# HalfSummer11/CAPTRA

Measured on AMD Instinct MI355X. Metric: tracked frames/sec (4096-pt clouds), higher is better.
Workload: dtype f32; 1 GPU; NOCS-REAL275-shaped rigid category 'bottle' (1 part, symmetric), 4096 pts/frame, batch=32 trajectories per GPU, fp32 (BASELINE.json configs[1]); points=4096, trajectories_per_gpu=32, distinct_clouds_per_gpu=32, parallelism=dp1 (trajectory-sharded, RCCL all-gather of poses), weights=seeded default_rng(7), real architecture (3.96 M params), physical-regime plants

## Files before the change

captra_amd/_lib.py:

```python
from __future__ import annotations

import contextlib
import ctypes as C
import threading
import os
from pathlib import Path

import torch

_PKG = Path(__file__).resolve().parent
LIB_PATH = Path(os.environ["CAPTRA_LIB"]) if os.environ.get("CAPTRA_LIB") else _PKG / "lib" / "libcaptra_hip.so"

_lib = None

_INT, _LL, _F, _P = C.c_int, C.c_longlong, C.c_float, C.c_void_p

_SIGNATURES = {
    "captra_furthest_point_sampling": [_INT, _INT, _INT, _P, _P, _P, _P],
    "captra_ball_query": [_INT, _INT, _INT, _F, _INT, _P, _P, _P, _P],
    "captra_group_points": [_INT, _INT, _INT, _INT, _INT, _P, _P, _P, _P],
    "captra_group_points_multi": [_INT, _INT, _INT, _P, _P, _P, _P, _P, _P, _P],
    "captra_group_points_grad": [_INT, _INT, _INT, _INT, _INT, _P, _P, _P, _P],
    "captra_group_points_grad_ws": [_INT, _INT, _INT, _INT, _INT, _P, _P, _P, _P, C.c_size_t, _P],
    "captra_three_interpolate_grad_ws": [_INT, _INT, _INT, _INT, _P, _P, _P, _P, _P, C.c_size_t, _P],
# ... 100 lines not shown
    "captra_packed_weight_floats": ([_INT, _INT], _LL),
    "captra_dense_bf16_image_bytes": ([_INT, _INT], _LL),
    "captra_gn_stats_bf16pm_tiles": ([_LL], _INT),
    "captra_dense_bf16_stats_tiles": ([_LL], _INT),
    "captra_dense_bf16_tile_stats_tiles": ([_LL], _INT),
    "captra_chain_bf16_image_bytes": ([_INT, _INT], _LL),
    "captra_dense_x6_image_bytes": ([_INT, _INT], _LL),
    "captra_sa_x6_image_bytes": ([_INT] * 4, _LL),
    "captra_chain_x6_image_bytes": ([_INT, _P, _P], _LL),
    "captra_sa_bf16_image_bytes": ([_INT] * 4, _LL),
    "captra_sa1_stream_scratch_bytes": ([_INT, _INT], _LL),
    "captra_sa1_stream_set_grid": ([_INT, _INT], None),
    "captra_sa1_stream_set_fine": ([_INT], None),
    "captra_sa1_stream_set_whole": ([_INT], None),
    "captra_neck_chain_set_split": ([_INT], None),
    "captra_image_members_set_split": ([_INT], None),
    "captra_query_and_group_set_shape": ([_INT, _INT], None),
    "captra_pointwise_mlp_gn_tiles": ([_INT, _INT, _LL], _INT),
    "captra_pointwise_mlp_gn_tiles_ex": ([_INT, _INT, _LL, _P], _INT),
}

_ENV_SWITCHES = {
    "CAPTRA_BF16_SHARED_AFFINE": ("captra_dense_bf16_set_shared_affine", ()),
    "CAPTRA_SA_BF16_VARIANT": ("captra_sa_bf16_set_variant", ()),
    "CAPTRA_FPS_DEFER": ("captra_fps_set_defer", ()),
    "CAPTRA_NN_SPLIT": ("captra_three_nn_set_split", ()),
    "CAPTRA_BQ_CPW": ("captra_ball_query_set_cpw", ()),
    "CAPTRA_SA_SPLIT": ("captra_sa_fused_set_split", ()),
    "CAPTRA_HEAD_PERSIST": ("captra_tile_bf16_set_persistent", ()),
    "CAPTRA_L1_FINE": ("captra_sa1_stream_set_fine", ()),
    "CAPTRA_L1_WHOLE": ("captra_sa1_stream_set_whole", ()),
    "CAPTRA_L1_GRID": ("captra_sa1_stream_set_grid", (1,)),
}


class CaptraHipError(RuntimeError):
    pass


class LaunchOpts(C.Structure):
    _fields_ = [("splitk_positions", _INT), ("sa_prezeroed", _INT), ("centre_m0", _INT), ("centre_mc", _INT), ("reserved_cus", _INT),
                ("dyn_slot", _P)]

# ... 146 lines not shown
```

captra_amd/csrc/sa_fused.hip:

```cpp
#include "common.h"
#include "wave_mlp.h"

namespace {


constexpr int SF_POS = 128;
constexpr int SF_BK = 16;
constexpr int SF_BM = 128;
constexpr int SF_MAXC = 256;

struct SaParams {
    int n, m, k, cfeat;
    int c1, c2, c3;
    const float *feat;
    const float *xyz_cn;
    const float *new_xyz;
    const int *idx;
    const float *w1, *b1, *w2, *b2, *w3, *b3;
    float *out;
    int out_ctotal, co_off;
};

template <int WN>
__device__ __forceinline__ void sa_prefetch_first(float (&pre)[16], const float *__restrict__ wt, int cin, int cout) {
// ... 222 lines not shown
    }
}

struct SwParams {
    int b, n, m, k;
    const float *feat, *xyz_cn, *new_xyz;
    const int *idx;
    const float *w1, *b1, *w2, *b2, *w3, *b3;
    float *out;
    int out_ctotal, co_off;
    const float *v1;
    unsigned long long *prof;
    int split;
    int m0, mc;
    int *dyn;
};

#define SW_TICK(slot)                                                         \
    if (CAPTRA_PROF_ON(p.prof)) {                                                  \
        const unsigned long long t_now = __builtin_amdgcn_s_memtime();        \
        if (lane == 0 && sampled) atomicAdd(p.prof + (slot), t_now - t_last); \
        t_last = t_now;                                                       \
    }

template <int CF, int C1, int NOUT, typename Next>
__device__ __forceinline__ void sw_layer1_gather(const SwParams &p, int b, int id, const float (&ctr)[3], const float *bias_lds,
                                                 float (&hout)[NOUT], int lane, Next next) {
    constexpr int CIN = CF + 3;
    using S = SwShape<CIN, C1>;
    constexpr int NT = S::NT;
// ... 240 lines not shown
#undef SL_LOAD_QUAD
#pragma unroll
        for (int tm = 0; tm < 2; ++tm)
            if (2 * ps + tm < S::NT) {
                if (LAST) sw_bfly_accumulate(acc[tm], zrun[2 * ps + tm], lane);
                else sw_mid_epilogue<NOUT>(acc[tm], 2 * ps + tm, hout);
            }
    }
}

template <int CF, int C1, int C2, int C3>
constexpr int sl_lds_floats() {
    return SlShape<CF + 3, C1>::FLOATS + SlShape<C1, C2>::FLOATS + SlShape<C2, C3>::FLOATS + pad32c(C1) + pad32c(C2) + pad32c(C3);
}

template <int CF, int C1, int C2, int C3>
__device__ __forceinline__ void sl_body(const SwParams &p, const int blk, const int nblk) {
    constexpr int CIN1 = CF + 3;
    static_assert(CIN1 <= 8, "LDS-weight variant is for the small-input scales");
    using S1 = SlShape<CIN1, C1>;
    using S2 = SlShape<C1, C2>;
    using S3 = SlShape<C2, C3>;
    extern __shared__ __attribute__((aligned(16))) float lds[];
    float *wl1 = lds, *wl2 = wl1 + S1::FLOATS, *wl3 = wl2 + S2::FLOATS;
    float *bias1 = wl3 + S3::FLOATS, *bias2 = bias1 + pad32c(C1), *bias3 = bias2 + pad32c(C2);
    const int tid = threadIdx.x, lane = tid & 63;
    const int wave = __builtin_amdgcn_readfirstlane(tid >> 6);

    const int nwaves = nblk * SL_WAVES, gid = blk * SL_WAVES + wave;
    const int ncentres = p.b * p.mc;
// ... 14 lines not shown
            else if (row < CIN1) v = p.xyz_cn[((size_t)tb * 3 + (row - CF)) * p.n + id_] - (row - CF == 0 ? c_[0] : (row - CF == 1 ? c_[1] : c_[2]));
            x_[j] = v;
        }
    };
    const bool split = p.split != 0;
    const int ssh = __builtin_ctz((unsigned)nslices);
    int task = gid;
    int c = split ? gid >> ssh : gid, sl = split ? gid & (nslices - 1) : 0;
    int c_next = gid + nwaves;
    const bool dyn = p.dyn != nullptr && !split && nslices > 1;
    int dyn_raw = 0;
    if (dyn) {
        if (lane == 0) dyn_raw = atomicAdd(p.dyn, 1);
        c = __builtin_amdgcn_readfirstlane(dyn_raw);
    }
    int id = 0;
    float ctr[3] = {0.f, 0.f, 0.f};
    if (c < ncentres) {
        id = load_ids(c, sl);
        load_ctr(c, ctr);
    }
    sl_stage_weights<CIN1, C1>(wl1, p.w1, tid);
    sl_stage_weights<C1, C2>(wl2, p.w2, tid);
    sl_stage_weights<C2, C3>(wl3, p.w3, tid);
    for (int e = tid; e < pad32c(C1); e += SL_WAVES * 64) bias1[e] = p.b1[e];
    for (int e = tid; e < pad32c(C2); e += SL_WAVES * 64) bias2[e] = p.b2[e];
    for (int e = tid; e < pad32c(C3); e += SL_WAVES * 64) bias3[e] = p.b3[e];
    __syncthreads();

    float x1[S1::KST];
#pragma unroll
    for (int j = 0; j < S1::KST; ++j) x1[j] = 0.f;
    if (c < ncentres) gather_x1(c, id, ctr, x1);
    int zrun[S3::NT];
    const bool sampled = blk % 16 == 0;
    unsigned long long t_last = CAPTRA_PROF_ON(p.prof) ? __builtin_amdgcn_s_memtime() : 0ull;
    while (c < ncentres) {
        if (sl == 0 || split) {
#pragma unroll
            for (int t = 0; t < S3::NT; ++t) zrun[t] = 0;
        }
        const bool last_slice = split || sl + 1 == nslices;
        if (dyn) {
            if (sl == 0 && lane == 0) dyn_raw = atomicAdd(p.dyn, 1);
            if (last_slice) c_next = __builtin_amdgcn_readfirstlane(dyn_raw);
        }
        const int cn = split ? (task + nwaves) >> ssh : (last_slice ? c_next : c), sn = split ? (task + nwaves) & (nslices - 1) : (last_slice ? 0 : sl + 1);
        const bool has_next = cn < ncentres;
        int id_n = 0;
        float ctr_n[3] = {ctr[0], ctr[1], ctr[2]};
        if (has_next) {
            id_n = load_ids(cn, sn);
            if (last_slice) load_ctr(cn, ctr_n);
        }
        float h1[S2::KST], h2[S3::KST], none[1];
        float x1_n[S1::KST];
#pragma unroll
        for (int j = 0; j < S1::KST; ++j) x1_n[j] = 0.f;
        SW_TICK(0)
        sl_layer<CIN1, C1, false>(wl1, bias1, x1, h1, zrun, lane);
        SW_TICK(1)
        sl_layer<C1, C2, false>(wl2, bias2, h1, h2, zrun, lane);
        if (has_next) gather_x1(cn, id_n, ctr_n, x1_n);
        SW_TICK(2)
        sl_layer<C2, C3, true>(wl3, bias3, h2, none, zrun, lane);
        SW_TICK(3)
        if (CAPTRA_PROF_ON(p.prof) && lane == 0 && sampled) atomicAdd(p.prof + 9, 1ull);
        if (last_slice) {
            const int tb = c / p.mc, centre = p.m0 + c - tb * p.mc;
            const int r = lane & 15;
            const int row0 = 8 * (r >> 2) + (r & 3) + 4 * (lane >> 5);
            float *op = p.out + ((size_t)tb * p.out_ctotal + p.co_off + row0) * p.m + centre;
#pragma unroll
            for (int t = 0; t < S3::NT; ++t) {
                const float v = sw_bfly_finish(zrun[t]);
                if ((lane & 16) == 0 && 32 * t + row0 < C3) {
                    if (split) atomicMax(reinterpret_cast<int *>(op + (size_t)32 * t * p.m), __float_as_int(v));
                    else op[(size_t)32 * t * p.m] = v;
                }
            }
            if (!dyn) c_next += nwaves;
// ... 18 lines not shown
    const int blk = (int)blockIdx.x;
    if (blk < q.g0) sl_body<CF, 32, 32, 64>(q.s[0], blk, q.g0);
    else if (blk < q.g0 + q.g1) sl_body<CF, 64, 64, 128>(q.s[1], blk - q.g0, q.g1);
    else sl_body<CF, 64, 96, 128>(q.s[2], blk - q.g0 - q.g1, (int)gridDim.x - q.g0 - q.g1);
}

}

static CAPTRA_KNOB int g_sa_wn = 0;
extern "C" void captra_sa_fused_set_wn(int wn) { g_sa_wn = wn; }
static CAPTRA_KNOB int g_sa_mode = 0;
extern "C" void captra_sa_fused_set_mode(int mode) { g_sa_mode = mode; }
static CAPTRA_KNOB int g_sa_split = 1;
extern "C" void captra_sa_fused_set_split(int v) { g_sa_split = v; }
int captra_sa_split_knob() { return g_sa_split; }
struct SlRecord {
    SwParams q;
    unsigned grid;
    int code, cf, lds;
    void (*launch)(const SwParams &, unsigned, int, hipStream_t);
};
struct SlCollect {
    SlRecord rec[3];
    int n = 0;
    alignas(16) unsigned char sp[1024];
};
template <int CF, int C1, int C2, int C3>
static void sl_launch_one(const SwParams &q, unsigned grid, int lds, hipStream_t s) {
    CAPTRA_LAUNCH("sa_scale_fused", (sa_wave_lds_kernel<CF, C1, C2, C3>), dim3(grid), dim3(SL_WAVES * 64), lds, s, q);
}
// ... 50 lines not shown
                               const float *w3, const float *b3, float *out, int out_ctotal, int co_off,
                               const captra_launch_opts *opts, SlCollect *col, captra_stream_t stream) {
    if (b < 0 || n < 1 || m < 0 || k < 1 || cfeat < 0 || c1 < 1 || c2 < 1 || c3 < 1) return -1;
    if (cfeat > 0 && feat == nullptr) return -1;
    if (out_ctotal < co_off + c3 || co_off < 0) return -1;
    if (k % 32 != 0 || 128 % k != 0 || c1 > SF_MAXC || c2 > SF_MAXC || c3 > SF_MAXC) return -2;
    if (b == 0 || m == 0) return 0;
    SaParams p;
    p.n = n; p.m = m; p.k = k; p.cfeat = cfeat; p.c1 = c1; p.c2 = c2; p.c3 = c3;
    p.feat = feat; p.xyz_cn = xyz_cn; p.new_xyz = new_xyz; p.idx = idx;
    p.w1 = w1; p.b1 = b1; p.w2 = w2; p.b2 = b2; p.w3 = w3; p.b3 = b3;
    p.out = out; p.out_ctotal = out_ctotal; p.co_off = co_off; 
    if (g_sa_mode != 1) {
        SwParams q;
        q.b = b; q.n = n; q.m = m; q.k = k; q.feat = feat; q.xyz_cn = xyz_cn; q.new_xyz = new_xyz; q.idx = idx;
        q.w1 = w1; q.b1 = b1; q.w2 = w2; q.b2 = b2; q.w3 = w3; q.b3 = b3; q.out = out; q.out_ctotal = out_ctotal; q.co_off = co_off; q.v1 = nullptr; q.prof = g_sa_prof; q.split = 0; q.dyn = nullptr;
        const long long Lw = (long long)m * k;
        dim3 gridw((unsigned)((Lw + SF_POS - 1) / SF_POS), b);
#define SL_CASE(CF_, C1_, C2_, C3_)                                                                                   \
    if (g_sa_mode != 2 && cfeat == CF_ && c1 == C1_ && c2 == C2_ && c3 == C3_ && k % 32 == 0 && (long long)b * m < (1ll << 30)) { \
        constexpr auto kern = sa_wave_lds_kernel<CF_, C1_, C2_, C3_>;                                                  \
        constexpr int lds_bytes = sl_lds_floats<CF_, C1_, C2_, C3_>() * 4;                                             \
        if (int e = captra_allow_lds<kern>(lds_bytes)) return e;                                                       \
         \
        const int resident = captra_blocks_per_cu<kern>(SL_WAVES * 64, lds_bytes) * captra_free_cus(opts);             \
        int wm0, wmc;                                                                                                  \
        (void)captra_centre_window(opts, m, &wm0, &wmc);                                                               \
        if (wmc == 0) return 0;                                                                                        \
        q.m0 = wm0; q.mc = wmc;                                                                                        \
        const long long centres = (long long)b * wmc;                     \
         \
// ... 92 lines not shown
    const int ferr = sl_collect_flush(col, (hipStream_t)stream);
    return err != 0 ? err : ferr;
}

extern "C" int captra_sa_scale_pre(int b, int n, int m, int k, int cfeat, int c1, int c2, int c3, const float *v1,
                                   const float *xyz_cn, const float *new_xyz, const int *idx, const float *w1,
                                   const float *w2, const float *b2, const float *w3, const float *b3, float *out,
                                   int out_ctotal, int co_off, captra_stream_t stream) {
    if (b < 0 || n < 1 || m < 0 || k < 1 || cfeat < 1 || c1 < 1 || c2 < 1 || c3 < 1 || v1 == nullptr) return -1;
    if (out_ctotal < co_off + c3 || co_off < 0) return -1;
    if (k % 32 != 0 || 128 % k != 0) return -2;
    if ((long long)c1 * n * 4 >= (1ll << 31)) return -2;
    SwParams q;
    q.b = b; q.n = n; q.m = m; q.k = k; q.feat = nullptr; q.xyz_cn = xyz_cn; q.new_xyz = new_xyz; q.idx = idx;
    q.w1 = w1; q.b1 = b2 ; q.w2 = w2; q.b2 = b2; q.w3 = w3; q.b3 = b3;
    q.out = out; q.out_ctotal = out_ctotal; q.co_off = co_off; q.v1 = v1; q.prof = g_sa_prof; q.split = 0; q.dyn = nullptr;
    const long long Lw = (long long)m * k;
    dim3 gridw((unsigned)((Lw + SF_POS - 1) / SF_POS), b);
#define SWP_CASE(CF_, C1_, C2_, C3_)                                                                                       \
    if (cfeat == CF_ && c1 == C1_ && c2 == C2_ && c3 == C3_) {                                                             \
        if (b == 0 || m == 0) return 0;                                                                                    \
        CAPTRA_LAUNCH("sa_scale_fused", (sa_wave_kernel<CF_, C1_, C2_, C3_, true>), gridw, dim3(256), 0, (hipStream_t)stream, q); \
        return captra_last_error();                                                                                        \
    }
    SWP_CASE(320, 128, 128, 256)
    SWP_CASE(320, 128, 196, 256)
#undef SWP_CASE
    return -2;
}
```

captra_amd/csrc/sa_pipe.hip:

```cpp
#include "wave_mlp.h"

namespace {

constexpr int SP_POS = 128;

struct SpParams {
    int b, n, m, k;
    const float *v1pm;
    const float *xyz_cn;
    const float *new_xyz;
    const int *idx;
    const float *w1;
    const float *w2, *b2, *w3, *b3;
    float *out;
    int out_ctotal, co_off;
    unsigned long long *prof;
    int split;
    int *dyn;
};

#define SP_TICK(slot)                                                           \
    if (CAPTRA_PROF_ON(p.prof)) {                                                    \
        const unsigned long long t_now = __builtin_amdgcn_s_memtime();          \
        if (lane == 0 && sampled) atomicAdd(p.prof + (slot), t_now - t_last);   \
        t_last = t_now;                                                         \
    }

template <int NOUT>
__device__ __forceinline__ void sp_mid_unit(const f32x16 &acc, int t, int q, float (&hout)[NOUT]) {
    unsigned a[4];
#pragma unroll
    for (int i = 0; i < 4; ++i) {
        const int x = __float_as_int(acc[4 * q + i]);
// ... 145 lines not shown
    float at[2][NT1];
    {
        const __amdgpu_buffer_rsrc_t rw = __builtin_amdgcn_make_buffer_rsrc((void *)p.w1, 0, S1::KP * S1::LDW * 4, 0x00020000);
        const int voff_w = (half * S1::LDW + (lane & 31)) * 4;
#pragma unroll
        for (int jj = 0; jj < 2; ++jj)
#pragma unroll
            for (int t = 0; t < NT1; ++t)
                at[jj][t] = __builtin_bit_cast(float, __builtin_amdgcn_raw_buffer_load_b32(rw, voff_w, ((CF + 2 * jj) * S1::LDW + 32 * t) * 4, 0));
    }
    __syncthreads();

    const int nwaves = nblk * 4, gid = blk * 4 + wave;
    const int ncentres = p.b * p.m;
    const int nslices = p.k / 32;
    int id = 0;
    float bt[2] = {0.f, 0.f};
    float4 g4[NT1][4];
    auto load_id = [&](int c, int sl) { return p.idx[(size_t)c * p.k + sl * 32 + (lane & 31)]; };
    auto load_rest = [&](int c, int id_, float (&bt_)[2], float4 (&g_)[NT1][4]) {
        const int tb = c / p.m;
        const float *cp = p.new_xyz + (size_t)c * 3;
#pragma unroll
        for (int jj = 0; jj < 2; ++jj) {
            const int a = 2 * jj + half;
            bt_[jj] = a < 3 ? p.xyz_cn[((size_t)tb * 3 + a) * p.n + id_] - cp[a] : 0.f;
        }
        const float4 *vp = reinterpret_cast<const float4 *>(p.v1pm + ((size_t)tb * p.n + id_) * C1 + 4 * half);
#pragma unroll
        for (int t = 0; t < NT1; ++t)
#pragma unroll
// ... 4 lines not shown
    unsigned long long t_last = CAPTRA_PROF_ON(p.prof) ? __builtin_amdgcn_s_memtime() : 0ull;
    float s[3][16];
    constexpr int START3 = S2::STEPS % 3;
    constexpr int NEXT2 = (START3 + S3::STEPS) % 3;
    int zrun[S3::NT];
    const bool split = p.split != 0;
    const int ssh = __builtin_ctz((unsigned)nslices);
    int task = gid;
    int c = split ? gid >> ssh : gid, sl = split ? gid & (nslices - 1) : 0;
    const bool dyn = p.dyn != nullptr && !split && nslices > 1;
    int dyn_raw = 0, c_next = gid + nwaves;
    if (dyn) {
        if (lane == 0) dyn_raw = atomicAdd(p.dyn, 1);
        c = __builtin_amdgcn_readfirstlane(dyn_raw);
    }
    if (c < ncentres) {
        sw_first_set<C1, C2>(s[NEXT2], p.w2, lane);
        id = load_id(c, sl);
        load_rest(c, id, bt, g4);
    }
    while (c < ncentres) {
        if (sl == 0 || split) {
#pragma unroll
            for (int t = 0; t < S3::NT; ++t) zrun[t] = 0;
        }
        const bool last_slice = split || sl + 1 == nslices;
        if (dyn) {
            if (sl == 0 && lane == 0) dyn_raw = atomicAdd(p.dyn, 1);
            if (last_slice) c_next = __builtin_amdgcn_readfirstlane(dyn_raw);
        } else {
            c_next = c + nwaves;
        }
        const int cn = split ? (task + nwaves) >> ssh : (last_slice ? c_next : c), sn = split ? (task + nwaves) & (nslices - 1) : (last_slice ? 0 : sl + 1);
        const bool has_next = cn < ncentres;
        int id_n = 0;

        float h1[S2::KST], h2[S3::KST], none[1];
        SP_TICK(0)
        if (NEXT2 != 0) {
#pragma unroll
            for (int i = 0; i < 16; ++i) s[0][i] = s[NEXT2][i];
        }
        {
            f32x16 acc[NT1];
#pragma unroll
            for (int t = 0; t < NT1; ++t)
#pragma unroll
                for (int q = 0; q < 4; ++q) {
                    acc[t][4 * q + 0] = g4[t][q].x; acc[t][4 * q + 1] = g4[t][q].y;
                    acc[t][4 * q + 2] = g4[t][q].z; acc[t][4 * q + 3] = g4[t][q].w;
// ... 41 lines not shown
            racc[1] = bias_lds[C2M + 2 * half + 1];
            rem_load(0);
        }
        __builtin_amdgcn_sched_barrier(0);
        SP_TICK(1)
        sp_layer<C1, C2M, false, 0, REM ? S2::NSETS : 0, 5>(p.w2, bias_lds, h1, h2, s, zrun, lane,
                                   [&](float (&dst)[16]) { sw_first_set<C2, C3>(dst, p.w3, lane); },
                                   [&](int g) {
                                       if (g == 1 && has_next) id_n = load_id(cn, sn);
                                       if (g + 1 < S2::NSETS) rem_load(g + 1);
                                   },
                                   [&](int g) { rem_step(g); });
        SP_TICK(2)
        sp_layer<C2, C3, true, START3, 0, 0>(p.w3, bias_lds + 256, h2, none, s, zrun, lane,
                                       [&](float (&dst)[16]) { sw_first_set<C1, C2>(dst, p.w2, lane); },
                                       [&](int g) { if (g == 2 && has_next) load_rest(cn, id_n, bt, g4); },
                                       [](int) {});
        id = id_n;
        SP_TICK(3)
        if (CAPTRA_PROF_ON(p.prof) && lane == 0 && sampled) atomicAdd(p.prof + 9, 1ull);
        if (last_slice) {
            const int tb = c / p.m, centre = c - tb * p.m;
            const int r = lane & 15;
            const int row0 = 8 * (r >> 2) + (r & 3) + 4 * half;
            float *op = p.out + ((size_t)tb * p.out_ctotal + p.co_off + row0) * p.m + centre;
#pragma unroll
            for (int t = 0; t < S3::NT; ++t) {
                const float v = sw_bfly_finish(zrun[t]);
                if ((lane & 16) == 0 && 32 * t + row0 < C3) {
                    if (split) atomicMax(reinterpret_cast<int *>(op + (size_t)32 * t * p.m), __float_as_int(v));
                    else op[(size_t)32 * t * p.m] = v;
                }
            }
// ... 8 lines not shown
__global__ __launch_bounds__(256) __attribute__((amdgpu_waves_per_eu(1, 1))) void sa_wave_pipe_kernel(SpParams p) {
    sp_body<CF, C1, C2, C3>(p, (int)blockIdx.x, (int)gridDim.x);
}

struct Sp2Params { SpParams s[2]; int g0; };
__global__ __launch_bounds__(256) __attribute__((amdgpu_waves_per_eu(1, 1))) void sa_wave_pipe2_kernel(Sp2Params q) {
    const int blk = (int)blockIdx.x;
    if (blk < q.g0) sp_body<320, 128, 128, 256>(q.s[0], blk, q.g0);
    else sp_body<320, 128, 196, 256>(q.s[1], blk - q.g0, (int)gridDim.x - q.g0);
}

}

extern unsigned long long *captra_sa_prof_ptr();
extern int captra_sa_split_knob();
extern int *captra_sa_dyn_slot(const captra_launch_opts *o, hipStream_t stream);

struct SpRecord { SpParams q; unsigned grid; int code; };
struct SpCollect { SpRecord rec[2]; int n; };
void captra_sp_collect_init(void *buf, size_t bytes) {
    static_assert(sizeof(SpCollect) <= 1024, "SlCollect::sp (sa_fused.hip) holds an SpCollect");
    if (buf != nullptr && bytes >= sizeof(SpCollect)) static_cast<SpCollect *>(buf)->n = 0;
}
int captra_sp_collect_flush(void *buf, hipStream_t s) {
    SpCollect &c = *static_cast<SpCollect *>(buf);
    const int n = c.n;
    c.n = 0;
    if (n == 2 && c.rec[0].code == 0 && c.rec[1].code == 1 && c.rec[0].q.dyn == nullptr && c.rec[1].q.dyn == nullptr) {
        Sp2Params q2;
        q2.s[0] = c.rec[0].q; q2.s[1] = c.rec[1].q; q2.g0 = (int)c.rec[0].grid;
// ... 10 lines not shown
int captra_sa_scale_pre_pm_impl(int b, int n, int m, int k, int cfeat, int c1, int c2, int c3, const float *v1pm,
                                const float *xyz_cn, const float *new_xyz, const int *idx, const float *w1,
                                const float *w2, const float *b2, const float *w3, const float *b3, float *out,
                                int out_ctotal, int co_off, const captra_launch_opts *opts, void *spbuf, captra_stream_t stream) {
    SpCollect *col = static_cast<SpCollect *>(spbuf);
    if (b < 0 || n < 1 || m < 0 || k < 1 || cfeat < 1 || c1 < 1 || c2 < 1 || c3 < 1 || v1pm == nullptr) return -1;
    if (out_ctotal < co_off + c3 || co_off < 0) return -1;
    if (k % 32 != 0 || 128 % k != 0) return -2;
    const long long L = (long long)m * k;
    if (L % SP_POS != 0 || (long long)c1 * n * 4 >= (1ll << 31) || (long long)b * L >= (1ll << 31)) return -2;
    if (b == 0 || m == 0) return 0;
    SpParams q;
    q.b = b; q.n = n; q.m = m; q.k = k; q.v1pm = v1pm; q.xyz_cn = xyz_cn; q.new_xyz = new_xyz; q.idx = idx;
    q.w1 = w1; q.w2 = w2; q.b2 = b2; q.w3 = w3; q.b3 = b3; q.out = out; q.out_ctotal = out_ctotal; q.co_off = co_off;
    q.prof = captra_sa_prof_ptr();
    const int cus = captra_free_cus(opts);
    const long long centres = (long long)b * m;
    if (centres >= (1ll << 30)) return -2;
    const int split_knob = captra_sa_split_knob();
    q.split = (split_knob != 0 && k > 32 && (split_knob == 2 || centres < 4ll * cus)) ? 1 : 0;
    const long long wgs = ((q.split ? centres * (k / 32) : centres) + 3) / 4;
    const unsigned grid = (unsigned)(wgs < cus ? wgs : cus);
    q.dyn = (!q.split && k > 32 && wgs > 1 && col == nullptr) ? captra_sa_dyn_slot(opts, (hipStream_t)stream) : nullptr;
    if (q.split && !(opts != nullptr && opts->sa_prezeroed)) {
        if (b <= 8 && ((size_t)c3 * m * 4) % 16 == 0 && (reinterpret_cast<uintptr_t>(out + (size_t)co_off * m) & 15) == 0 && ((size_t)out_ctotal * m * 4) % 16 == 0) {
            for (int bb = 0; bb < b; ++bb) (void)captra_zero_async(out + ((size_t)bb * out_ctotal + co_off) * m, (size_t)c3 * m * 4, (hipStream_t)stream);
        } else {
            (void)hipMemset2DAsync(out + (size_t)co_off * m, (size_t)out_ctotal * m * 4, 0, (size_t)c3 * m * 4, b, (hipStream_t)stream);
        }
    }
// ... 30 lines not shown
```

captra_amd/csrc/wave_mlp.h:

```cpp
#pragma once
#include "common.h"
#include "wave_ops.h"

namespace {

typedef float f32x16 __attribute__((ext_vector_type(16)));

constexpr int pad32c(int c) { return (c + 31) / 32 * 32; }
constexpr int pad128c(int c) { return (c + 127) / 128 * 128; }

constexpr int SW_KS = 8;

template <int CIN, int COUT>
struct SwShape {
    static constexpr int KST = (CIN + 1) / 2;
    static constexpr int NSETS = (KST + SW_KS - 1) / SW_KS;
    static constexpr int NT = (COUT + 31) / 32;
    static constexpr int NPASS = (NT + 1) / 2;
    static constexpr int STEPS = NPASS * NSETS;
    static constexpr int LDW = pad128c(COUT), KP = pad32c(CIN);
};

template <int CIN, int COUT>
struct SwFrag {
// ... 106 lines not shown
    }
#pragma unroll
    for (int m = 0; m < 2; ++m) {
        const int own = b2 ? v[2 * m + 1] : v[2 * m], oth = b2 ? v[2 * m] : v[2 * m + 1];
        const int p = dpp_keep<0x104, 0xF, 0x5>(own, oth);
        const int q = dpp_keep<0x114, 0xF, 0xA>(p, oth);
        u[m] = imax(own, q);
    }
    const int own = b3 ? u[1] : u[0], oth = b3 ? u[0] : u[1];
    zrun = imax(zrun, imax_dpp<0x128>(own, oth));
}
__device__ __forceinline__ float sw_bfly_finish(int zrun) {
    return __int_as_float(imax(zrun, __builtin_amdgcn_ds_swizzle(zrun, 0x401F)));
}


enum { SW_EPI_MID = 0, SW_EPI_MAX = 1, SW_EPI_STORE = 2 };

struct SwStore {
    float *y = nullptr;
    long long ld = 0;
    bool col_ok = true;
    int act = 1;
};

template <int COUT>
__device__ __forceinline__ void sw_store_epilogue(const f32x16 &acc, int t, const SwStore &st, int lane) {
    if (!st.col_ok) return;
    float *yp = st.y + (size_t)(32 * t + 4 * (lane >> 5)) * st.ld + (lane & 31);
#pragma unroll
// ... 51 lines not shown
```

captra_amd/fused.py:

```python
from __future__ import annotations

import contextlib
import ctypes as C
import os
import threading

import numpy as np
import torch

from . import _lib as L
from .fold import PackedLinear

ACT_NONE, ACT_RELU, ACT_SIGMOID_M05 = 0, 1, 2

WORK = {"on": False, "flops": {}, "bytes": {}}


def work_reset(on: bool = True) -> None:
    WORK["on"] = on
    WORK["flops"].clear()
    WORK["bytes"].clear()


def _work(name: str, flops: float = 0.0, nbytes: float = 0.0) -> None:
    if WORK["on"]:
        WORK["flops"][name] = WORK["flops"].get(name, 0.0) + flops
        WORK["bytes"][name] = WORK["bytes"].get(name, 0.0) + nbytes


def canonicalize(pts, mean, rot, trans, scale, num_parts: int = 1, want_cn=True, want_n3=True, want_planes=False):
    B, _, N = pts.shape
    Q = B * num_parts
    mean = mean.reshape(B, 3).contiguous()
    rot = rot.reshape(Q, 3, 3).contiguous()
    trans = trans.reshape(Q, 3).contiguous()
    scale = scale.reshape(Q).contiguous()
    L.require_device(pts, mean, rot, trans, scale)
    out_cn = torch.empty(Q, 3, N, dtype=torch.float32, device=pts.device) if want_cn else None
    out_n3 = torch.empty(Q, N, 3, dtype=torch.float32, device=pts.device) if want_n3 else None
    if want_planes:
        planes = torch.empty(Q, 3, (N + 255) // 256 * 256, dtype=torch.float32, device=pts.device)
        with torch.cuda.device(pts.device):
# ... 737 lines not shown


def sa_scale_pre_pm(v1pm, xyz_cn, new_xyz_n3, idx, layers, out, co_off, cfeat, jobs=None):
    l1, l2, l3 = layers
    L.require_device(v1pm, xyz_cn, new_xyz_n3, idx, out)
    B, _, N = xyz_cn.shape
    _, M, K = idx.shape
    if jobs is not None:
        jobs.append(L.SaScaleJob(1, B, N, M, K, cfeat, l1.cout, l2.cout, l3.cout, L.ptr(v1pm), L.ptr(xyz_cn), L.ptr(new_xyz_n3), L.ptr(idx),
                                 L.ptr(l1.wt), None, L.ptr(l2.wt), L.ptr(l2.bias), L.ptr(l3.wt), L.ptr(l3.bias), L.ptr(out), out.shape[1], co_off))
    else:
        with torch.cuda.device(xyz_cn.device):
            L.call("captra_sa_scale_pre_pm", B, N, M, K, cfeat, l1.cout, l2.cout, l3.cout, L.ptr(v1pm), L.ptr(xyz_cn),
                   L.ptr(new_xyz_n3), L.ptr(idx), L.ptr(l1.wt), L.ptr(l2.wt), L.ptr(l2.bias), L.ptr(l3.wt), L.ptr(l3.bias),
                   L.ptr(out), out.shape[1], co_off)
    _work("sa_scale_fused", flops=2.0 * B * M * K * (3 * l1.cout + l1.cout * l2.cout + l2.cout * l3.cout),
          nbytes=4.0 * B * (l1.cout * N + 3 * N + M * K + 3 * M + l3.cout * M))
    return out


def sa_scale_pre(v1, xyz_cn, new_xyz_n3, idx, layers, out, co_off, cfeat):
    l1, l2, l3 = layers
    L.require_device(v1, xyz_cn, new_xyz_n3, idx, out)
    B, _, N = xyz_cn.shape
    _, M, K = idx.shape
    with torch.cuda.device(xyz_cn.device):
        L.call("captra_sa_scale_pre", B, N, M, K, cfeat, l1.cout, l2.cout, l3.cout, L.ptr(v1), L.ptr(xyz_cn),
               L.ptr(new_xyz_n3), L.ptr(idx), L.ptr(l1.wt), L.ptr(l2.wt), L.ptr(l2.bias), L.ptr(l3.wt), L.ptr(l3.bias),
               L.ptr(out), out.shape[1], co_off)
    _work("sa_scale_fused", flops=2.0 * B * M * K * (3 * l1.cout + l1.cout * l2.cout + l2.cout * l3.cout),
          nbytes=4.0 * B * (l1.cout * N + 3 * N + M * K + 3 * M + l3.cout * M))
# ... 263 lines not shown
    L.require_device(feat, xyz_cn, new_xyz_n3, idx, out, *[t for l in layers for t in (l.wt, l.bias)])
    B, _, N = xyz_cn.shape
    _, M, K = idx.shape
    cfeat = 0 if feat is None else feat.shape[1]
    l1, l2, l3 = layers
    (w1, b1), (w2, b2), (w3, b3) = (l1.wt, l1.bias), (l2.wt, l2.bias), (l3.wt, l3.bias)
    c1, c2, c3 = l1.cout, l2.cout, l3.cout
    assert l1.cin == cfeat + 3 and l2.cin == c1 and l3.cin == c2
    if jobs is not None:
        jobs.append(L.SaScaleJob(0, B, N, M, K, cfeat, c1, c2, c3, L.ptr(feat), L.ptr(xyz_cn), L.ptr(new_xyz_n3), L.ptr(idx), L.ptr(w1), L.ptr(b1),
                                 L.ptr(w2), L.ptr(b2), L.ptr(w3), L.ptr(b3), L.ptr(out), out.shape[1], co_off))
    else:
        with torch.cuda.device(xyz_cn.device):
            L.call("captra_sa_scale_fused", B, N, M, K, cfeat, c1, c2, c3, L.ptr(feat), L.ptr(xyz_cn), L.ptr(new_xyz_n3),
                   L.ptr(idx), L.ptr(w1), L.ptr(b1), L.ptr(w2), L.ptr(b2), L.ptr(w3), L.ptr(b3), L.ptr(out), out.shape[1], co_off)
    _work("sa_scale_fused", flops=2.0 * B * M * K * ((cfeat + 3) * c1 + c1 * c2 + c2 * c3),
          nbytes=4.0 * B * ((cfeat + 3) * N + M * K + 3 * M + c3 * M))
    return out


def three_nn_weights(unknown_n3, known_n3):
    L.require_device(unknown_n3, known_n3)
    B, N, _ = unknown_n3.shape
    S = known_n3.shape[1]
    idx = torch.empty(B, N, 3, dtype=torch.int32, device=unknown_n3.device)
    w = torch.empty(B, N, 3, dtype=torch.float32, device=unknown_n3.device)
    with torch.cuda.device(unknown_n3.device):
        L.call("captra_three_nn_weights", B, N, S, L.ptr(unknown_n3), L.ptr(known_n3), L.ptr(idx), L.ptr(w))
    _work("three_nn_weights", nbytes=B * (12.0 * N + 12.0 * S + 24.0 * N))
    return idx, w

# ... 29 lines not shown
```

include/captra_hip.h:

```cpp
#ifndef CAPTRA_HIP_H
#define CAPTRA_HIP_H

#include <stddef.h>

#ifdef __cplusplus
extern "C" {
#endif

typedef void *captra_stream_t;

typedef struct captra_launch_opts {
    int splitk_positions;
    int sa_prezeroed;
    int centre_m0, centre_mc;
    int reserved_cus;
    int *dyn_slot;
} captra_launch_opts;


int captra_furthest_point_sampling(int b, int n, int m, const float *xyz, float *temp, int *idx,
                                   captra_stream_t stream);

int captra_ball_query(int b, int n, int m, float radius, int nsample, const float *new_xyz,
                      const float *xyz, int *idx, captra_stream_t stream);
// ... 339 lines not shown

const char *captra_error_string(int err);
const char *captra_version(void);
void captra_prof_enable(int on);
void captra_prof_reset(void);
int captra_prof_read(const char *name, double *total_ms, long long *launches);
int captra_prof_names(char *buf, int buflen);

void captra_fps_set_waves(int waves);
void captra_fps_set_pruned_min(int n);
void captra_fps_set_stats(unsigned long long *dev_counters);
void captra_fps_set_variant(int v);
void captra_sa_fused_set_mode(int mode);
void captra_sa_fused_set_wn(int wn);
void captra_sa_fused_set_prof(unsigned long long *dev_counters);
void captra_pw_set_direct(int on);
void captra_ball_query_set_prune(int on);
void captra_pw_set_occupancy(int occ);
void captra_pw_set_dbg(int v);
void captra_pw_set_pair(int on);
void captra_sa1_stream_set_grid(int grid, int prio);
void captra_sa1_stream_set_fine(int centres);
void captra_sa1_stream_set_whole(int windows);
void captra_sa_bf16_set_variant(int v);
void captra_image_members_set_split(int n);
void captra_neck_chain_set_split(int n);
void captra_query_and_group_set_shape(int mcb, int cc);
void captra_group_set_shape(int lds_kb, int ccmax, int ppb);

#ifdef __cplusplus
// ... 4 lines not shown
```

Measured before the change: 5984 frames/s.

## Skip ball-query padding slices in fused SA MLP kernels

Ball query pads each neighbour row by repeating its first index. Any 32-wide slice after the first that holds only that repeated index cannot change the max-pool, so it is treated as dead. Both the LDS-weight and pipelined SA kernels now build a per-centre live-slice mask from ballots over tail indices and jump past dead slices, or mark split tasks idle. This removes MLP work on duplicate neighbours, at the cost of extra index loads and ballots per centre and more control flow. It is on by default and can be turned off with an env knob.

```diff
diff --git a/captra_amd/_lib.py b/captra_amd/_lib.py
--- a/captra_amd/_lib.py
+++ b/captra_amd/_lib.py
@@ -138,6 +138,7 @@
     "captra_sa1_stream_set_fine": ([_INT], None),
     "captra_sa1_stream_set_whole": ([_INT], None),
     "captra_neck_chain_set_split": ([_INT], None),
+    "captra_sa_set_skip_padded": ([_INT], None),
     "captra_image_members_set_split": ([_INT], None),
     "captra_query_and_group_set_shape": ([_INT, _INT], None),
     "captra_pointwise_mlp_gn_tiles": ([_INT, _INT, _LL], _INT),
@@ -151,6 +152,7 @@
     "CAPTRA_NN_SPLIT": ("captra_three_nn_set_split", ()),
     "CAPTRA_BQ_CPW": ("captra_ball_query_set_cpw", ()),
     "CAPTRA_SA_SPLIT": ("captra_sa_fused_set_split", ()),
+    "CAPTRA_SA_SKIP": ("captra_sa_set_skip_padded", ()),
     "CAPTRA_HEAD_PERSIST": ("captra_tile_bf16_set_persistent", ()),
     "CAPTRA_L1_FINE": ("captra_sa1_stream_set_fine", ()),
     "CAPTRA_L1_WHOLE": ("captra_sa1_stream_set_whole", ()),
diff --git a/captra_amd/csrc/sa_fused.hip b/captra_amd/csrc/sa_fused.hip
--- a/captra_amd/csrc/sa_fused.hip
+++ b/captra_amd/csrc/sa_fused.hip
@@ -260,6 +260,7 @@
     int split;
     int m0, mc;
     int *dyn;
+    int skip;
 };
 
 #define SW_TICK(slot)                                                         \
@@ -530,6 +531,8 @@
     return SlShape<CF + 3, C1>::FLOATS + SlShape<C1, C2>::FLOATS + SlShape<C2, C3>::FLOATS + pad32c(C1) + pad32c(C2) + pad32c(C3);
 }
 
+constexpr bool sl_skips_padding(int c1, int c2) { return c1 + c2 <= 128; }
+
 template <int CF, int C1, int C2, int C3>
 __device__ __forceinline__ void sl_body(const SwParams &p, const int blk, const int nblk) {
     constexpr int CIN1 = CF + 3;
@@ -574,11 +577,23 @@
         if (lane == 0) dyn_raw = atomicAdd(p.dyn, 1);
         c = __builtin_amdgcn_readfirstlane(dyn_raw);
     }
+    constexpr bool SKIPS = sl_skips_padding(C1, C2);
+    const bool skip = SKIPS && p.skip != 0 && nslices > 1;
+    const unsigned all_slices = (1u << nslices) - 1u;
+    unsigned live = all_slices;
+    bool idle = false;
+    auto row_of = [&](int c_) { return p.idx + (size_t)crow(c_) * p.k; };
     int id = 0;
     float ctr[3] = {0.f, 0.f, 0.f};
     if (c < ncentres) {
         id = load_ids(c, sl);
         load_ctr(c, ctr);
+        if constexpr (SKIPS) {
+            int ta, tb;
+            sw_load_tail_ids(row_of(c), p.k, lane, ta, tb);
+            if (skip && split) idle = sl > 0 && sw_slice_is_padding(id, sw_tail_entry0(tb));
+            if (skip && !split) live = sw_live_of_tail(ta, tb, p.k);
+        }
     }
     sl_stage_weights<CIN1, C1>(wl1, p.w1, tid);
     sl_stage_weights<C1, C2>(wl2, p.w2, tid);
@@ -596,16 +611,29 @@
     const bool sampled = blk % 16 == 0;
     unsigned long long t_last = CAPTRA_PROF_ON(p.prof) ? __builtin_amdgcn_s_memtime() : 0ull;
     while (c < ncentres) {
+        if (idle) {
+            task += nwaves; c = task >> ssh; sl = task & (nslices - 1);
+            idle = false;
+            if (c < ncentres) {
+                id = load_ids(c, sl);
+                idle = sl > 0 && sw_slice_is_padding(id, row_of(c)[0]);
+                load_ctr(c, ctr);
+                if (!idle) gather_x1(c, id, ctr, x1);
+            }
+            continue;
+        }
         if (sl == 0 || split) {
 #pragma unroll
             for (int t = 0; t < S3::NT; ++t) zrun[t] = 0;
         }
-        const bool last_slice = split || sl + 1 == nslices;
+        const unsigned rest = split ? 0u : live >> (sl + 1);
+        const bool last_slice = rest == 0u;
         if (dyn) {
             if (sl == 0 && lane == 0) dyn_raw = atomicAdd(p.dyn, 1);
             if (last_slice) c_next = __builtin_amdgcn_readfirstlane(dyn_raw);
         }
-        const int cn = split ? (task + nwaves) >> ssh : (last_slice ? c_next : c), sn = split ? (task + nwaves) & (nslices - 1) : (last_slice ? 0 : sl + 1);
+        const int cn = split ? (task + nwaves) >> ssh : (last_slice ? c_next : c);
+        const int sn = split ? (task + nwaves) & (nslices - 1) : (last_slice ? 0 : sl + 1 + __builtin_ctz(rest));
         const bool has_next = cn < ncentres;
         int id_n = 0;
         float ctr_n[3] = {ctr[0], ctr[1], ctr[2]};
@@ -621,10 +649,20 @@
         sl_layer<CIN1, C1, false>(wl1, bias1, x1, h1, zrun, lane);
         SW_TICK(1)
         sl_layer<C1, C2, false>(wl2, bias2, h1, h2, zrun, lane);
-        if (has_next) gather_x1(cn, id_n, ctr_n, x1_n);
+        int ta = 0, tb = 0;
+        if (has_next) {
+            gather_x1(cn, id_n, ctr_n, x1_n);
+            if constexpr (SKIPS) sw_load_tail_ids(row_of(cn), p.k, lane, ta, tb);
+        }
         SW_TICK(2)
         sl_layer<C2, C3, true>(wl3, bias3, h2, none, zrun, lane);
         SW_TICK(3)
+        if constexpr (SKIPS) {
+            const unsigned live_n = sw_live_of_tail(ta, tb, p.k);
+            const bool pad_n = sw_slice_is_padding(id_n, sw_tail_entry0(tb));
+            if (last_slice) live = (skip && has_next) ? live_n : all_slices;
+            idle = split && skip && has_next && sn > 0 && pad_n;
+        }
         if (CAPTRA_PROF_ON(p.prof) && lane == 0 && sampled) atomicAdd(p.prof + 9, 1ull);
         if (last_slice) {
             const int tb = c / p.mc, centre = p.m0 + c - tb * p.mc;
@@ -673,6 +711,9 @@
 static CAPTRA_KNOB int g_sa_split = 1;
 extern "C" void captra_sa_fused_set_split(int v) { g_sa_split = v; }
 int captra_sa_split_knob() { return g_sa_split; }
+static CAPTRA_KNOB int g_sa_skip = 1;
+extern "C" void captra_sa_set_skip_padded(int on) { g_sa_skip = on != 0 ? 1 : 0; }
+int captra_sa_skip_knob() { return g_sa_skip; }
 struct SlRecord {
     SwParams q;
     unsigned grid;
@@ -753,7 +794,7 @@
     if (g_sa_mode != 1) {
         SwParams q;
         q.b = b; q.n = n; q.m = m; q.k = k; q.feat = feat; q.xyz_cn = xyz_cn; q.new_xyz = new_xyz; q.idx = idx;
-        q.w1 = w1; q.b1 = b1; q.w2 = w2; q.b2 = b2; q.w3 = w3; q.b3 = b3; q.out = out; q.out_ctotal = out_ctotal; q.co_off = co_off; q.v1 = nullptr; q.prof = g_sa_prof; q.split = 0; q.dyn = nullptr;
+        q.w1 = w1; q.b1 = b1; q.w2 = w2; q.b2 = b2; q.w3 = w3; q.b3 = b3; q.out = out; q.out_ctotal = out_ctotal; q.co_off = co_off; q.v1 = nullptr; q.prof = g_sa_prof; q.split = 0; q.dyn = nullptr; q.skip = g_sa_skip;
         const long long Lw = (long long)m * k;
         dim3 gridw((unsigned)((Lw + SF_POS - 1) / SF_POS), b);
 #define SL_CASE(CF_, C1_, C2_, C3_)                                                                                   \
@@ -876,7 +917,7 @@
     SwParams q;
     q.b = b; q.n = n; q.m = m; q.k = k; q.feat = nullptr; q.xyz_cn = xyz_cn; q.new_xyz = new_xyz; q.idx = idx;
     q.w1 = w1; q.b1 = b2 ; q.w2 = w2; q.b2 = b2; q.w3 = w3; q.b3 = b3;
-    q.out = out; q.out_ctotal = out_ctotal; q.co_off = co_off; q.v1 = v1; q.prof = g_sa_prof; q.split = 0; q.dyn = nullptr;
+    q.out = out; q.out_ctotal = out_ctotal; q.co_off = co_off; q.v1 = v1; q.prof = g_sa_prof; q.split = 0; q.dyn = nullptr; q.skip = g_sa_skip;
     const long long Lw = (long long)m * k;
     dim3 gridw((unsigned)((Lw + SF_POS - 1) / SF_POS), b);
 #define SWP_CASE(CF_, C1_, C2_, C3_)                                                                                       \
diff --git a/captra_amd/csrc/sa_pipe.hip b/captra_amd/csrc/sa_pipe.hip
--- a/captra_amd/csrc/sa_pipe.hip
+++ b/captra_amd/csrc/sa_pipe.hip
@@ -17,6 +17,7 @@
     unsigned long long *prof;
     int split;
     int *dyn;
+    int skip;
 };
 
 #define SP_TICK(slot)                                                           \
@@ -192,7 +193,6 @@
     const int nwaves = nblk * 4, gid = blk * 4 + wave;
     const int ncentres = p.b * p.m;
     const int nslices = p.k / 32;
-    int id = 0;
     float bt[2] = {0.f, 0.f};
     float4 g4[NT1][4];
     auto load_id = [&](int c, int sl) { return p.idx[(size_t)c * p.k + sl * 32 + (lane & 31)]; };
@@ -227,26 +227,50 @@
         if (lane == 0) dyn_raw = atomicAdd(p.dyn, 1);
         c = __builtin_amdgcn_readfirstlane(dyn_raw);
     }
+    const bool skip = p.skip != 0 && nslices > 1;
+    const unsigned all_slices = (1u << nslices) - 1u;
+    unsigned live = all_slices;
+    bool idle = false;
+    auto row_of = [&](int c_) { return p.idx + (size_t)c_ * p.k; };
+    int id = 0;
     if (c < ncentres) {
         sw_first_set<C1, C2>(s[NEXT2], p.w2, lane);
         id = load_id(c, sl);
+        {
+            int ta, tb;
+            sw_load_tail_ids(row_of(c), p.k, lane, ta, tb);
+            if (skip && split) idle = sl > 0 && sw_slice_is_padding(id, sw_tail_entry0(tb));
+            if (skip && !split) live = sw_live_of_tail(ta, tb, p.k);
+        }
         load_rest(c, id, bt, g4);
     }
     while (c < ncentres) {
+        if (idle) {
+            task += nwaves; c = task >> ssh; sl = task & (nslices - 1);
+            idle = false;
+            if (c < ncentres) {
+                id = load_id(c, sl);
+                idle = sl > 0 && sw_slice_is_padding(id, row_of(c)[0]);
+                if (!idle) load_rest(c, id, bt, g4);
+            }
+            continue;
+        }
         if (sl == 0 || split) {
 #pragma unroll
             for (int t = 0; t < S3::NT; ++t) zrun[t] = 0;
         }
-        const bool last_slice = split || sl + 1 == nslices;
+        const unsigned rest = split ? 0u : live >> (sl + 1);
+        const bool last_slice = rest == 0u;
         if (dyn) {
             if (sl == 0 && lane == 0) dyn_raw = atomicAdd(p.dyn, 1);
             if (last_slice) c_next = __builtin_amdgcn_readfirstlane(dyn_raw);
         } else {
             c_next = c + nwaves;
         }
-        const int cn = split ? (task + nwaves) >> ssh : (last_slice ? c_next : c), sn = split ? (task + nwaves) & (nslices - 1) : (last_slice ? 0 : sl + 1);
+        const int cn = split ? (task + nwaves) >> ssh : (last_slice ? c_next : c);
+        const int sn = split ? (task + nwaves) & (nslices - 1) : (last_slice ? 0 : sl + 1 + __builtin_ctz(rest));
         const bool has_next = cn < ncentres;
-        int id_n = 0;
+        int id_n = 0, ta = 0, tb = 0;
 
         float h1[S2::KST], h2[S3::KST], none[1];
         SP_TICK(0)
@@ -318,9 +342,19 @@
         SP_TICK(2)
         sp_layer<C2, C3, true, START3, 0, 0>(p.w3, bias_lds + 256, h2, none, s, zrun, lane,
                                        [&](float (&dst)[16]) { sw_first_set<C1, C2>(dst, p.w2, lane); },
-                                       [&](int g) { if (g == 2 && has_next) load_rest(cn, id_n, bt, g4); },
+                                       [&](int g) {
+                                           if (g == 2 && has_next) {
+                                               load_rest(cn, id_n, bt, g4);
+                                               sw_load_tail_ids(row_of(cn), p.k, lane, ta, tb);
+                                           }
+                                       },
                                        [](int) {});
-        id = id_n;
+        {
+            const unsigned live_n = sw_live_of_tail(ta, tb, p.k);
+            const bool pad_n = sw_slice_is_padding(id_n, sw_tail_entry0(tb));
+            if (last_slice) live = (skip && has_next) ? live_n : all_slices;
+            idle = split && skip && has_next && sn > 0 && pad_n;
+        }
         SP_TICK(3)
         if (CAPTRA_PROF_ON(p.prof) && lane == 0 && sampled) atomicAdd(p.prof + 9, 1ull);
         if (last_slice) {
@@ -359,6 +393,7 @@
 
 extern unsigned long long *captra_sa_prof_ptr();
 extern int captra_sa_split_knob();
+extern int captra_sa_skip_knob();
 extern int *captra_sa_dyn_slot(const captra_launch_opts *o, hipStream_t stream);
 
 struct SpRecord { SpParams q; unsigned grid; int code; };
@@ -399,6 +434,7 @@
     q.b = b; q.n = n; q.m = m; q.k = k; q.v1pm = v1pm; q.xyz_cn = xyz_cn; q.new_xyz = new_xyz; q.idx = idx;
     q.w1 = w1; q.w2 = w2; q.b2 = b2; q.w3 = w3; q.b3 = b3; q.out = out; q.out_ctotal = out_ctotal; q.co_off = co_off;
     q.prof = captra_sa_prof_ptr();
+    q.skip = captra_sa_skip_knob();
     const int cus = captra_free_cus(opts);
     const long long centres = (long long)b * m;
     if (centres >= (1ll << 30)) return -2;
diff --git a/captra_amd/csrc/wave_mlp.h b/captra_amd/csrc/wave_mlp.h
--- a/captra_amd/csrc/wave_mlp.h
+++ b/captra_amd/csrc/wave_mlp.h
@@ -144,6 +144,23 @@
     return __int_as_float(imax(zrun, __builtin_amdgcn_ds_swizzle(zrun, 0x401F)));
 }
 
+__device__ __forceinline__ bool sw_slice_is_padding(int ids, int id0) { return __ballot(ids != id0) == 0ull; }
+__device__ __forceinline__ void sw_load_tail_ids(const int *row, int k, int lane, int &ta, int &tb) {
+    const int oa = 32 + (k > 64 ? lane : (lane & 31)), ob = lane < 32 ? 96 + lane : 0;
+    ta = row[oa < k ? oa : k - 1];
+    tb = row[ob < k ? ob : k - 1];
+}
+__device__ __forceinline__ int sw_tail_entry0(int tb) { return __builtin_amdgcn_readlane(tb, 32); }
+__device__ __forceinline__ unsigned sw_live_of_tail(int ta, int tb, int k) {
+    const int e0 = sw_tail_entry0(tb);
+    const unsigned long long da = __ballot(ta != e0);
+    const unsigned db = (unsigned)__ballot(tb != e0);
+    unsigned live = 1u;
+    if (k > 32) live |= (unsigned)da != 0u ? 2u : 0u;
+    if (k > 64) live |= ((da >> 32) != 0ull ? 4u : 0u) | (db != 0u ? 8u : 0u);
+    return live;
+}
+
 
 enum { SW_EPI_MID = 0, SW_EPI_MAX = 1, SW_EPI_STORE = 2 };
 
diff --git a/captra_amd/fused.py b/captra_amd/fused.py
--- a/captra_amd/fused.py
+++ b/captra_amd/fused.py
@@ -26,6 +26,16 @@
     if WORK["on"]:
         WORK["flops"][name] = WORK["flops"].get(name, 0.0) + flops
         WORK["bytes"][name] = WORK["bytes"].get(name, 0.0) + nbytes
+
+
+def sa_positions_computed(idx, skips: bool = True) -> float:
+    B, M, K = idx.shape
+    if not (WORK["on"] and skips and K > 32 and os.environ.get("CAPTRA_SA_SKIP", "1") != "0") or torch.cuda.is_current_stream_capturing():
+        return float(B) * M * K
+    slices = idx.reshape(B, M, K // 32, 32)
+    padding = (slices == slices[:, :, :1, :1]).all(dim=3)
+    padding[:, :, 0] = False
+    return 32.0 * float((~padding).sum().item())
 
 
 def canonicalize(pts, mean, rot, trans, scale, num_parts: int = 1, want_cn=True, want_n3=True, want_planes=False):
@@ -793,7 +803,7 @@
             L.call("captra_sa_scale_pre_pm", B, N, M, K, cfeat, l1.cout, l2.cout, l3.cout, L.ptr(v1pm), L.ptr(xyz_cn),
                    L.ptr(new_xyz_n3), L.ptr(idx), L.ptr(l1.wt), L.ptr(l2.wt), L.ptr(l2.bias), L.ptr(l3.wt), L.ptr(l3.bias),
                    L.ptr(out), out.shape[1], co_off)
-    _work("sa_scale_fused", flops=2.0 * B * M * K * (3 * l1.cout + l1.cout * l2.cout + l2.cout * l3.cout),
+    _work("sa_scale_fused", flops=2.0 * sa_positions_computed(idx) * (3 * l1.cout + l1.cout * l2.cout + l2.cout * l3.cout),
           nbytes=4.0 * B * (l1.cout * N + 3 * N + M * K + 3 * M + l3.cout * M))
     return out
 
@@ -1087,7 +1097,8 @@
         with torch.cuda.device(xyz_cn.device):
             L.call("captra_sa_scale_fused", B, N, M, K, cfeat, c1, c2, c3, L.ptr(feat), L.ptr(xyz_cn), L.ptr(new_xyz_n3),
                    L.ptr(idx), L.ptr(w1), L.ptr(b1), L.ptr(w2), L.ptr(b2), L.ptr(w3), L.ptr(b3), L.ptr(out), out.shape[1], co_off)
-    _work("sa_scale_fused", flops=2.0 * B * M * K * ((cfeat + 3) * c1 + c1 * c2 + c2 * c3),
+    skips = cfeat + 3 <= 8 and c1 + c2 <= 128
+    _work("sa_scale_fused", flops=2.0 * sa_positions_computed(idx, skips) * ((cfeat + 3) * c1 + c1 * c2 + c2 * c3),
           nbytes=4.0 * B * ((cfeat + 3) * N + M * K + 3 * M + c3 * M))
     return out
 
diff --git a/include/captra_hip.h b/include/captra_hip.h
--- a/include/captra_hip.h
+++ b/include/captra_hip.h
@@ -377,6 +377,7 @@
 void captra_sa_fused_set_mode(int mode);
 void captra_sa_fused_set_wn(int wn);
 void captra_sa_fused_set_prof(unsigned long long *dev_counters);
+void captra_sa_set_skip_padded(int on);
 void captra_pw_set_direct(int on);
 void captra_ball_query_set_prune(int on);
 void captra_pw_set_occupancy(int occ);
```

After: 5947 frames/s. About the same (-0.6%).
